# NethermindEth/cairo_zstd

Hardware: AMD Instinct MI355X
Metric: decompressed MB/s (whole node), 128 KiB-block batch (higher is better)
Workload: dtype u8

## Files before the change

cairo_zstd_amd/csrc/czstd_chain.hip:

```cpp
#include "czstd_dict.h"

#ifndef CZC_SLOTS
#define CZC_SLOTS 10
#endif
#define CZC_LPS 4
static_assert(CZC_SLOTS * CZC_LPS <= 64, "quads of one wave");
#define CZC_MAXSYM 64
#define CZC_RING 512u
#define CZC_STEPS 32u
static_assert(((CZC_STEPS * 58u + 7u) / 8u + 12u) + 12u <= 256u + 12u, "a top-up adds at most 256 bytes: one must be enough for the next group");
#define CZC_NEED ((CZC_STEPS * 58u + 7u) / 8u + 12u)
#define CZC_MAP_WORDS CZ_CHAIN_MAP_WORDS

#define CZC_E16(nb, base, xb) ((uint16_t)(((((1u << (9u - (nb))) | ((base) >> (nb))) << 6) | (xb))))
#define CZC_E16_IDLE 0x8000u

struct CzChainSlot {
    uint16_t t_ll[512], t_ml[512], t_of[256];
    union {
        struct {
            __attribute__((aligned(16))) uint8_t stage[256];
            int16_t probs[3][CZC_MAXSYM];
            uint16_t counters_ml[CZC_MAXSYM];
        };
// ... 118 lines not shown
    else if (since >= 16u) asm volatile("s_waitcnt vmcnt(16)" ::: "memory");
    else asm volatile("s_waitcnt vmcnt(0)" ::: "memory");
    asm volatile("v_accvgpr_read_b32 %0, a0\nv_accvgpr_read_b32 %1, a1\nv_accvgpr_read_b32 %2, a2\nv_accvgpr_read_b32 %3, a3\n"
                 "v_accvgpr_read_b32 %4, a4\nv_accvgpr_read_b32 %5, a5\nv_accvgpr_read_b32 %6, a6\nv_accvgpr_read_b32 %7, a7\n"
                 "v_accvgpr_read_b32 %8, a8\nv_accvgpr_read_b32 %9, a9\nv_accvgpr_read_b32 %10, a10\nv_accvgpr_read_b32 %11, a11\n"
                 "v_accvgpr_read_b32 %12, a12\nv_accvgpr_read_b32 %13, a13\nv_accvgpr_read_b32 %14, a14\nv_accvgpr_read_b32 %15, a15"
                 : "=v"(v[0].x), "=v"(v[0].y), "=v"(v[0].z), "=v"(v[0].w), "=v"(v[1].x), "=v"(v[1].y), "=v"(v[1].z), "=v"(v[1].w),
                   "=v"(v[2].x), "=v"(v[2].y), "=v"(v[2].z), "=v"(v[2].w), "=v"(v[3].x), "=v"(v[3].y), "=v"(v[3].z), "=v"(v[3].w)
                 :: "memory");
}
#else
struct CzcPre { uint4 v[CZC_PF]; };
__device__ static inline void czc_prefetch(CzcPre& pre, int has_slot, intptr_t lo, uintptr_t Sk, uintptr_t Ek) {
    const uint32_t j = (uint32_t)LANE & 3u;
    for (uint32_t r = 0; r < CZC_PF; r++) {
        const uint32_t c = j + r * CZC_LPS;
        if (has_slot) pre.v[r] = czc_load16((uintptr_t)lo - 16u * (c + 1), Sk, Ek);
    }
}
__device__ static inline void czc_pre_settle() { }
__device__ static inline void czc_pre_take(const CzcPre& pre, uint32_t, uint4* v) { for (uint32_t r = 0; r < CZC_PF; r++) v[r] = pre.v[r]; }
#endif
__device__ static inline void czc_commit(CzChainSlot& sk, int has_slot, int32_t old_lo, int32_t new_lo, const CzcPre& pre, uint32_t since) {
    const uint32_t j = (uint32_t)LANE & 3u;
    const uint32_t cnt = has_slot ? (uint32_t)(old_lo - new_lo) >> 4 : 0u;
    uint4 v[CZC_PF];
    czc_pre_take(pre, since, v);
#pragma unroll
    for (uint32_t r = 0; r < CZC_PF; r++) {
        const uint32_t c = j + r * CZC_LPS;
        if (c < cnt) {
            const uint32_t slot = ((uint32_t)old_lo - 16u * (c + 1)) & (CZC_RING - 1);
            *(uint4*)&sk.ring[slot] = v[r];
            if (slot == CZC_RING - 16) { *(uint32_t*)&sk.mirror[4] = v[r].y; *(uint32_t*)&sk.mirror[8] = v[r].z; *(uint32_t*)&sk.mirror[12] = v[r].w; }
        }
    }
}
__device__ static inline uint64_t czc_window(const CzChainSlot& sl, int32_t u) {
    const uint32_t ba = ((uint32_t)u >> 3) & (CZC_RING - 4), ph = (uint32_t)u & 31;
    const uint32_t w2 = *(const uint32_t*)(sl.ring + ba), w1 = *(const uint32_t*)(sl.ring + ba - 4), w0 = *(const uint32_t*)(sl.ring + ba - 8);
    const uint64_t hi = (((uint64_t)w2 << 32) | w1), lo = (((uint64_t)w1 << 32) | w0);
    const uint32_t h = ph ? (uint32_t)(hi >> ph) : w1, l = ph ? (uint32_t)(lo >> ph) : w0;
    return ((uint64_t)h << 32) | l;
}

struct CzcLane {
    uint32_t E;
    uint32_t S;
    int32_t  u;
    uint32_t ph;
    uint32_t w0, w1, w2;
    uint32_t slow;
};
struct CzcRole {
    const uint16_t* tb;
    const uint8_t* ringm8;
    uint32_t m1, m2;
    uint32_t sh;
    uint32_t lane0;
    uint32_t sbits;
};
#define CZC_QP(a, b, c, d) ((a) | ((b) << 2) | ((c) << 4) | ((d) << 6))
template <int CTRL> __device__ static inline uint32_t czc_qp(uint32_t v) { return (uint32_t)__builtin_amdgcn_update_dpp(0, (int)v, CTRL, 0xF, 0xF, true); }

__device__ static inline void czc_ring_words(CzcLane& c, const CzcRole& ro) {
    const uint8_t* ba = ro.ringm8 + (__builtin_amdgcn_ubfe((uint32_t)c.u, 5, 7) << 2);
    c.w0 = *(const uint32_t*)ba; c.w1 = *(const uint32_t*)(ba + 4); c.w2 = *(const uint32_t*)(ba + 8);
    c.ph = (uint32_t)c.u & 31u;
}
__device__ static inline uint32_t czc_bits32(const CzcRole& ro, uint32_t v) {
    const uint8_t* ba = ro.ringm8 + (__builtin_amdgcn_ubfe(v, 5, 7) << 2);
    return __builtin_amdgcn_alignbit(*(const uint32_t*)(ba + 8), *(const uint32_t*)(ba + 4), v & 31u);
}
#define CZC_WIDE_STEPS 16u
static_assert((CZC_WIDE_STEPS * 89u + 7u) / 8u + 12u <= CZC_NEED && CZC_STEPS % CZC_WIDE_STEPS == 0, "a redone asm group is whole wide groups, each within the staged bytes");
__device__ static inline void czc_step(CzcLane& c, const CzcRole& ro, CZ_GLOBAL uint64_t* rec, int act, int last, int store) {
    const uint32_t n = (uint32_t)__builtin_clz(c.E);
    const uint32_t x = __builtin_amdgcn_ubfe(c.E, 16, 5);
    const uint32_t p = (n << 8) + x;
    const uint32_t T = p + czc_qp<CZC_QP(1, 2, 0, 3)>(p) + czc_qp<CZC_QP(2, 0, 1, 3)>(p);
    const uint32_t t1 = czc_qp<CZC_QP(0, 0, 0, 0)>(p) & ro.m1, t2 = czc_qp<CZC_QP(1, 1, 1, 1)>(p) & ro.m2;
    const uint32_t incl = (t1 + t2 + p) >> 8;
    const uint32_t a_ = T & 0xFFu;
    const uint32_t xh = czc_bits32(ro, (uint32_t)c.u - a_);
    const uint32_t bits = __builtin_amdgcn_ubfe(xh, (0u - incl) & 31u, n);
    const uint32_t window = czc_bits32(ro, (uint32_t)c.u);
    const uint32_t cS = c.S << ro.sh;
    const uint32_t H = cS + czc_qp<CZC_QP(1, 2, 0, 3)>(cS) + czc_qp<CZC_QP(2, 0, 1, 3)>(cS);
    if (act) {
        if (store) *rec = a_ <= 32 ? ((uint64_t)window | ((uint64_t)H << 32))
                                   : ((uint64_t)((uint32_t)c.u - ro.sbits) | ((uint64_t)(H | CZC_REC_WIDE) << 32));
        if (last) c.u -= (int32_t)a_;
        else {
            c.S = (((c.E >> 22) << n) | bits) & 511u;
            c.E = (uint32_t)ro.tb[c.S] << 16;
            c.u -= (int32_t)(a_ + (T >> 8));
        }
        czc_ring_words(c, ro);
    }
}

#if defined(__HIP_DEVICE_COMPILE__)
#define CZC_ASM_STORE(OFF) "global_store_dwordx4 %[RP], v[120:123], off offset:" #OFF "\n"
#define CZC_ASM_RING01 "ds_read2_b32 v[124:125], v115 offset1:1\n"
#define CZC_ASM_LGKM_E "s_waitcnt lgkmcnt(2)\n"

#define CZC_ASM2_HEAD(WIN) \
    CZC_ASM_LGKM_E \
    "v_ffbh_u32 v100, %[E]\n" \
    "v_bfe_u32 v101, %[E], 16, 5\n" \
    "v_lshl_or_b32 v102, v100, 8, v101\n" \
    "v_lshrrev_b32 v131, 22, %[E]\n" \
    "v_and_b32_dpp v106, v100, %[M1] quad_perm:[0,0,0,0] row_mask:0xf bank_mask:0xf\n" \
    "v_and_b32_dpp v107, v100, %[M2] quad_perm:[1,1,1,1] row_mask:0xf bank_mask:0xf\n" \
    "v_add_u32_dpp v105, v102, v102 quad_perm:[1,2,0,3] row_mask:0xf bank_mask:0xf\n" \
    "v_add_u32_dpp v105, v102, v105 quad_perm:[2,0,1,3] row_mask:0xf bank_mask:0xf\n" \
    "v_add3_u32 v109, v106, v107, v105\n" \
    "s_waitcnt lgkmcnt(0)\n" \
    "v_alignbit_b32 " WIN ", %[W2], v125, %[U]\n" \
    "v_alignbit_b32 v128, v125, v124, %[U]\n" \
    "v_mov_b32 v129, " WIN "\n" \
    "v_lshlrev_b64 v[128:129], v109, v[128:129]\n" \
    "v_mov_b32 v130, v129\n" \
    "v_lshlrev_b64 v[132:133], v100, v[130:131]\n" \
    "v_lshl_add_u32 v117, v133, 1, %[TB]\n" \
    "ds_read_u16_d16_hi %[E], v117\n"
#define CZC_ASM2_TAIL(STORE, NEXTH) \
    STORE \
    "v_lshl_add_u32 v118, v133, %[SH], %[NK]\n" \
    "v_dot4c_i32_i8_e32 %[U], 0xffff, v105\n" \
    "v_max_u32_sdwa %[SLOW], %[SLOW], v105 dst_sel:DWORD dst_unused:UNUSED_PAD src0_sel:DWORD src1_sel:BYTE_0\n"    \
    "v_add_u32_dpp " NEXTH ", v118, v118 quad_perm:[1,2,0,3] row_mask:0xf bank_mask:0xf\n" \
    "v_add_u32_dpp " NEXTH ", v118, " NEXTH " quad_perm:[2,0,1,3] row_mask:0xf bank_mask:0xf\n" \
    "v_bfe_u32 v114, %[U], 5, 7\n" \
    "v_lshl_add_u32 v115, v114, 2, %[RB]\n" \
    CZC_ASM_RING01 \
    "ds_read_b32 %[W2], v115 offset:8\n"
#define CZC_ASM2_EVEN(OFF) CZC_ASM2_HEAD("v120") CZC_ASM2_TAIL("", "v123")
#define CZC_ASM2_ODD(OFF) CZC_ASM2_HEAD("v122") CZC_ASM2_TAIL(CZC_ASM_STORE(OFF), "v121")
#define CZC_ASM2_PAIR(A) CZC_ASM2_EVEN(A) CZC_ASM2_ODD(A)
__device__ static inline void czc_group_asm2(CzcLane& c, const CzcRole& ro, CZ_GLOBAL uint64_t* rec) {
    static_assert(CZC_STEPS == 32, "the asm block is unrolled for 32 steps");
    const uint32_t tb32 = (uint32_t)(uintptr_t)(__attribute__((address_space(3))) const uint16_t*)ro.tb;
    const uint32_t rb32 = (uint32_t)(uintptr_t)(__attribute__((address_space(3))) const uint8_t*)ro.ringm8;
    const uint32_t tbm = tb32 - 1024u, nk = 0u - (512u << ro.sh);
    c.S += 512u;
    asm volatile(
        "v_mov_b32 v124, %[W0]\n"
        "v_mov_b32 v125, %[W1]\n"
        "v_mov_b32 v133, %[S]\n"
        "v_lshl_add_u32 v118, %[S], %[SH], %[NK]\n"
        "s_nop 1\n"
        "v_add_u32_dpp v121, v118, v118 quad_perm:[1,2,0,3] row_mask:0xf bank_mask:0xf\n"
        "v_add_u32_dpp v121, v118, v121 quad_perm:[2,0,1,3] row_mask:0xf bank_mask:0xf\n"
        CZC_ASM2_PAIR(0) CZC_ASM2_PAIR(16) CZC_ASM2_PAIR(32) CZC_ASM2_PAIR(48) CZC_ASM2_PAIR(64) CZC_ASM2_PAIR(80) CZC_ASM2_PAIR(96) CZC_ASM2_PAIR(112)
        CZC_ASM2_PAIR(128) CZC_ASM2_PAIR(144) CZC_ASM2_PAIR(160) CZC_ASM2_PAIR(176) CZC_ASM2_PAIR(192) CZC_ASM2_PAIR(208) CZC_ASM2_PAIR(224) CZC_ASM2_PAIR(240)
        "s_waitcnt lgkmcnt(0)\n"
        "v_and_b32 %[PH], 31, %[U]\n"
        "v_mov_b32 %[W0], v124\n"
        "v_mov_b32 %[W1], v125\n"
        "v_mov_b32 %[S], v133\n"
        : [E] "+v"(c.E), [S] "+v"(c.S), [U] "+v"(c.u), [PH] "+v"(c.ph), [W0] "+v"(c.w0), [W1] "+v"(c.w1), [W2] "+v"(c.w2), [SLOW] "+v"(c.slow)
        : [TB] "v"(tbm), [RB] "v"(rb32), [M1] "v"(ro.m1 ? 0xFFu : 0u), [M2] "v"(ro.m2 ? 0xFFu : 0u), [SH] "v"(ro.sh), [NK] "v"(nk), [RP] "v"(rec)
        : "memory",
          "v100", "v101", "v102", "v105", "v106", "v107", "v109", "v114", "v115", "v117", "v118", "v120", "v121", "v122", "v123", "v124", "v125",
          "v128", "v129", "v130", "v131", "v132", "v133");
    c.S -= 512u;
}

#define CZC_ASMW_HEAD(WIN) \
    "s_waitcnt lgkmcnt(2)\n" \
    "v_ffbh_u32 v100, %[E]\n" \
    "v_and_or_b32 v101, %[E], %[XM], %[K64]\n" \
    "v_sub_u32 v102, v101, v100\n" \
    "v_lshrrev_b32 v103, 22, %[E]\n" \
    "v_sub_u32 v119, %[U], %[SB]\n"                \
    "v_add_u32_dpp v105, v102, v102 quad_perm:[1,2,0,3] row_mask:0xf bank_mask:0xf\n" \
    "v_and_b32_dpp v106, v102, %[M1] quad_perm:[0,0,0,0] row_mask:0xf bank_mask:0xf\n" \
    "v_and_b32_dpp v107, v102, %[M2] quad_perm:[1,1,1,1] row_mask:0xf bank_mask:0xf\n" \
    "v_add_u32_dpp v105, v102, v105 quad_perm:[2,0,1,3] row_mask:0xf bank_mask:0xf\n" \
    "v_add3_u32 v109, v106, v107, v102\n" \
    "v_bfe_u32 v108, v105, 16, 8\n" \
    "s_waitcnt lgkmcnt(0)\n" \
    "v_cmp_ge_u32 vcc, %[PH], v108\n" \
    "v_sub_u32 v110, %[PH], v108\n" \
    "v_alignbit_b32 " WIN ", v127, v126, %[PH]\n" \
    "v_cndmask_b32 v111, v126, v127, vcc\n" \
    "v_cndmask_b32 v112, v125, v126, vcc\n" \
    "v_cmp_gt_i32 vcc, %[N32], v110\n"             \
    "v_cmp_lt_u32_e64 s[12:13], 32, v108\n" \
    "s_nop 0\n" \
    "v_cndmask_b32 v111, v111, v125, vcc\n" \
    "v_cndmask_b32 v112, v112, v124, vcc\n" \
    "v_alignbit_b32 v113, v111, v112, v110\n" \
    "v_bfe_u32 v116, v113, v109, v100\n" \
    "v_lshl_or_b32 %[S], v103, v100, v116\n" \
    "v_lshl_add_u32 v117, %[S], 1, %[TB]\n" \
    "ds_read_u16_d16_hi %[E], v117\n"
#define CZC_ASMW_TAIL(STORE, WIN, H, NEXTH) \
    "v_cndmask_b32_e64 " WIN ", " WIN ", v119, s[12:13]\n" \
    "v_cndmask_b32_e64 v128, 0, %[FL], s[12:13]\n" \
    "v_or_b32 " H ", " H ", v128\n" \
    STORE \
    "v_lshl_add_u32 v118, %[S], %[SH], %[NK]\n" \
    "v_dot4c_i32_i8_e32 %[U], 0x01ff0001, v105\n" \
    "v_and_b32 v129, 31, v108\n" \
    "v_add_u32_dpp " NEXTH ", v118, v118 quad_perm:[1,2,0,3] row_mask:0xf bank_mask:0xf\n" \
    "v_add_u32_dpp " NEXTH ", v118, " NEXTH " quad_perm:[2,0,1,3] row_mask:0xf bank_mask:0xf\n" \
    "v_bfe_u32 v114, %[U], 5, 7\n" \
    "v_and_b32 %[PH], 31, %[U]\n" \
    "v_lshl_add_u32 v115, v114, 2, %[RB]\n" \
    "ds_read2_b32 v[124:125], v115 offset1:1\n" \
    "ds_read2_b32 v[126:127], v115 offset0:2 offset1:3\n"
#define CZC_ASMW_EVEN(OFF) CZC_ASMW_HEAD("v120") CZC_ASMW_TAIL("", "v120", "v121", "v123")
#define CZC_ASMW_ODD(OFF) CZC_ASMW_HEAD("v122") CZC_ASMW_TAIL(CZC_ASM_STORE(OFF), "v122", "v123", "v121")
#define CZC_ASMW_PAIR(A) CZC_ASMW_EVEN(A) CZC_ASMW_ODD(A)
__device__ static inline void czc_group_asm_wide(CzcLane& c, const CzcRole& ro, CZ_GLOBAL uint64_t* rec) {
    const uint32_t tb32 = (uint32_t)(uintptr_t)(__attribute__((address_space(3))) const uint16_t*)ro.tb;
    const uint32_t rb32 = (uint32_t)(uintptr_t)(__attribute__((address_space(3))) const uint8_t*)ro.ringm8 - 4u;
    const uint32_t tbm = tb32 - 1024u, nk = 0u - (512u << ro.sh), k64 = ro.lane0 ? 0x40000040u : 0x40u;
    c.S += 512u;
    asm volatile(
        "v_bfe_u32 v114, %[U], 5, 7\n"
        "v_lshl_add_u32 v115, v114, 2, %[RB]\n"
        "ds_read2_b32 v[124:125], v115 offset1:1\n"
        "ds_read2_b32 v[126:127], v115 offset0:2 offset1:3\n"
        "v_lshl_add_u32 v118, %[S], %[SH], %[NK]\n"
        "s_nop 1\n"
        "v_add_u32_dpp v121, v118, v118 quad_perm:[1,2,0,3] row_mask:0xf bank_mask:0xf\n"
        "v_add_u32_dpp v121, v118, v121 quad_perm:[2,0,1,3] row_mask:0xf bank_mask:0xf\n"
        CZC_ASMW_PAIR(0) CZC_ASMW_PAIR(16) CZC_ASMW_PAIR(32) CZC_ASMW_PAIR(48) CZC_ASMW_PAIR(64) CZC_ASMW_PAIR(80) CZC_ASMW_PAIR(96) CZC_ASMW_PAIR(112)
        CZC_ASMW_PAIR(128) CZC_ASMW_PAIR(144) CZC_ASMW_PAIR(160) CZC_ASMW_PAIR(176) CZC_ASMW_PAIR(192) CZC_ASMW_PAIR(208) CZC_ASMW_PAIR(224) CZC_ASMW_PAIR(240)
        "s_waitcnt lgkmcnt(0)\n"
        : [E] "+v"(c.E), [S] "+v"(c.S), [U] "+v"(c.u), [PH] "+v"(c.ph)
        : [TB] "v"(tbm), [RB] "v"(rb32), [M1] "v"(ro.m1 ? 0xFFu : 0u), [M2] "v"(ro.m2 ? 0xFFu : 0u), [SH] "v"(ro.sh), [NK] "v"(nk), [K64] "v"(k64),
          [SB] "v"(ro.sbits), [FL] "v"(CZC_REC_WIDE), [XM] "s"(0x1F0000u), [N32] "s"(-32), [RP] "v"(rec)
        : "memory", "vcc", "s12", "s13",
          "v100", "v101", "v102", "v103", "v105", "v106", "v107", "v108", "v109", "v110", "v111", "v112", "v113", "v114", "v115",
          "v116", "v117", "v118", "v119", "v120", "v121", "v122", "v123", "v124", "v125", "v126", "v127", "v128", "v129");
    c.S -= 512u;
    czc_ring_words(c, ro);
}
#endif

#ifdef CZ_PROFILE
#define CZC_PROF_ACC(i) do { const unsigned long long n_ = __builtin_amdgcn_s_memtime(); cprof[i] += n_ - ct_; ct_ = n_; } while (0)
#define CZC_PROF_CNT(i) do { cprof[i] += 1; } while (0)
#else
#define CZC_PROF_ACC(i) do { } while (0)
#define CZC_PROF_CNT(i) do { } while (0)
#endif
#define CZC_LO_DEAD (-(1 << 30))
#define CZC_NSEQ_DEAD 0xFFFFFFFFu
#if defined(__HIP_DEVICE_COMPILE__)
__device__ static inline bool czc_any(bool b) { return __builtin_amdgcn_ballot_w64(b) != 0; }
#else
__device__ static inline bool czc_any(bool b) { return __ballot(b ? 1 : 0) != 0; }
#endif
__device__ static inline uint32_t czc_q0(uint32_t v) { return (uint32_t)__shfl((int)v, LANE & ~3); }
__device__ static inline uint64_t czc_q0_64(uint64_t v) { return ((uint64_t)czc_q0((uint32_t)(v >> 32)) << 32) | czc_q0((uint32_t)v); }

struct CzsBlk { uint32_t type, blk_off, bsize;
                uint32_t lt, regen, lit_hdr, nseq, sbody, modes; };
struct CzsWalk { const uint8_t* src; uint64_t len, pos, end, h8; uint32_t h8sh, defined, has_checksum; int first, active, ok, have_tree; };
__device__ static inline uint64_t czs_ld8_issue(const uint8_t* src, uint64_t len, uint64_t at, uint32_t* sh) {
    const uint64_t a2 = at + 8 <= len ? at : len - 8;
    uint64_t v; __builtin_memcpy(&v, src + a2, 8);
    *sh = (uint32_t)(at - a2);
    return v;
}
__device__ static inline uint64_t czs_ld8_value(uint64_t raw, uint32_t sh) { return sh >= 8 ? 0 : raw >> (8 * sh); }
__device__ static inline uint64_t czs_ld8(const uint8_t* src, uint64_t len, uint64_t at) { uint32_t sh; const uint64_t v = czs_ld8_issue(src, len, at, &sh); return czs_ld8_value(v, sh); }
__device__ static inline void czs_begin(CzsWalk& w, const uint8_t* src, uint64_t len, int valid) {
    w.src = src; w.len = len; w.pos = 0; w.end = 0; w.h8 = 0; w.h8sh = 8; w.defined = 0; w.has_checksum = 0; w.first = 1; w.active = 0; w.ok = 0; w.have_tree = 0;
    if (!valid || len < 8 || len >= 0xFFFFFFF0ull) return;
    const uint64_t h0 = czs_ld8(src, len, 0);
    const uint32_t magic = (uint32_t)h0;
    const uint32_t d = (uint32_t)(h0 >> 32) & 0xFF;
    const uint32_t single = (d >> 5) & 1, didf = d & 3, dl = didf == 3 ? 4 : didf, flag = d >> 6;
    const uint32_t fl = flag == 0 ? (single ? 1u : 0u) : flag == 1 ? 2u : flag == 2 ? 4u : 8u;
    const uint32_t hl = 5 + (single ? 0 : 1) + dl + fl;
    if (magic != 0xFD2FB528u || len < hl) return;
    if (!single) { const uint32_t wd = (uint32_t)(h0 >> 40) & 0xFF; const uint64_t base = 1ull << (10 + (wd >> 3)); if (base + (base / 8) * (wd & 7) >= 4123168604160ull) return; }
    w.pos = hl; w.active = 1; w.has_checksum = (d >> 2) & 1; w.h8 = czs_ld8_issue(src, len, hl, &w.h8sh);
}
__device__ static inline void czs_dict_check(CzsWalk& w, const cz_dict_entry* dicts, uint32_t ndicts) {
    if (!w.active) return;
    const uint64_t h0 = czs_ld8(w.src, w.len, 0);
    const uint32_t d = (uint32_t)(h0 >> 32) & 0xFF, didf = d & 3, dl = didf == 3 ? 4 : didf, at = 5 + (((d >> 5) & 1) ? 0 : 1);
    uint32_t id = (uint32_t)(h0 >> (8 * at));
    if (at + dl > 8) id |= (uint32_t)(czs_ld8(w.src, w.len, 8) << (8 * (8 - at)));
    id = dl == 0 ? 0u : (dl == 4 ? id : id & ((1u << (8 * dl)) - 1u));
    if (cz_dict_find(dicts, ndicts, id) == CZ_DICT_UNKNOWN) { w.active = 0; w.ok = 0; }
}
__device__ static inline int czs_next(CzsWalk& w, uint32_t chain_min_nseq, CzsBlk& b) {
    const uint8_t* src = w.src; const uint64_t len = w.len;
    if (!w.active) return 0;
    do {
        uint64_t pos = w.pos;
        if (pos == ~0ull) { w.active = 0; w.ok = 1; return 0; }
        if (len - pos < 3) break;
        const uint64_t h = czs_ld8_value(w.h8, w.h8sh);
        const uint32_t b0 = (uint32_t)h & 0xFF, b1 = (uint32_t)(h >> 8) & 0xFF, b2 = (uint32_t)(h >> 16) & 0xFF;
        const uint32_t type = (b0 >> 1) & 3, size = (b0 >> 3) | (b1 << 5) | (b2 << 13), blast = b0 & 1;
        if (type == 3 || size > 128u * 1024u) break;
        const uint64_t body = pos + 3; const uint32_t content = type == 1 ? 1u : size;
        if (len - body < content) break;
        w.pos = blast ? ~0ull : body + content;
        if (blast) w.end = body + content;
        else w.h8 = czs_ld8_issue(src, len, body + content, &w.h8sh);
        b.type = type; b.blk_off = (uint32_t)body; b.bsize = size; b.lt = 0; b.regen = 0; b.lit_hdr = 0; b.nseq = 0; b.sbody = 0; b.modes = 0;
        if (type != 2) return 1;
        if (size == 0) break;
        const uint32_t l0 = (uint32_t)(h >> 24) & 0xFF, lt = l0 & 3, fmt = (l0 >> 2) & 3;
        const uint32_t need = lt <= 1 ? ((fmt == 0 || fmt == 2) ? 1u : (fmt == 1 ? 2u : 3u)) : (fmt <= 1 ? 3u : (fmt == 2 ? 4u : 5u));
        if (size < need) break;
        const uint32_t l1 = need > 1 ? (uint32_t)(h >> 32) & 0xFF : 0, l2 = need > 2 ? (uint32_t)(h >> 40) & 0xFF : 0, l3 = need > 3 ? (uint32_t)(h >> 48) & 0xFF : 0, l4 = need > 4 ? (uint32_t)(h >> 56) & 0xFF : 0;
        uint32_t upper, regen;
        if (lt <= 1) { regen = (fmt == 0 || fmt == 2) ? l0 >> 3 : (fmt == 1 ? (l0 >> 4) + (l1 << 4) : (l0 >> 4) + (l1 << 4) + (l2 << 12)); upper = lt == 1 ? 1u : regen; }
        else {
            regen = fmt <= 1 ? (l0 >> 4) + ((l1 & 0x3f) << 4) : (fmt == 2 ? (l0 >> 4) + (l1 << 4) + ((l2 & 3) << 12) : (l0 >> 4) + (l1 << 4) + ((l2 & 0x3f) << 12));
            upper = fmt <= 1 ? (l1 >> 6) + (l2 << 2) : (fmt == 2 ? (l2 >> 2) + (l3 << 6) : (l2 >> 6) + (l3 << 2) + (l4 << 10));
        }
        if (size - need < upper) break;
        if (lt == 3 && !w.have_tree) break;
        if (lt == 2) w.have_tree = 1;
        const uint32_t so = need + upper, sl_ = size - so;
        if (sl_ == 0) break;
        const uint64_t sq = czs_ld8(src, len, body + so);
        const uint32_t s0 = (uint32_t)sq & 0xFF, s1 = (uint32_t)(sq >> 8) & 0xFF, s2 = (uint32_t)(sq >> 16) & 0xFF;
        uint32_t n = 0, hb = 0;
        if (s0 == 0) { }
        else if (s0 <= 127) { if (sl_ < 2) break; n = s0; hb = 1; }
        else if (s0 <= 254) { if (sl_ < 3) break; n = ((s0 - 128) << 8) + s1; hb = 2; }
        else { if (sl_ < 4) break; n = s1 + (s2 << 8) + 0x7F00u; hb = 3; }
        b.lt = lt; b.regen = regen; b.lit_hdr = need;
        if (!n) return 1;
        if (w.first && n < chain_min_nseq) break;
        b.nseq = n; b.modes = (uint32_t)(sq >> (8 * hb)) & 0xFF; b.sbody = so + hb + 1;
        int undefined = 0;
        for (int t = 0; t < 3; t++) {
// ... 205 lines not shown
        const unsigned long long wm = __ballot(wx);
        if (wm) {
            uint32_t base = 0;
            if (LANE == __ffsll((long long)wm) - 1) base = atomicAdd(&a.scan_ctl[206], (uint32_t)__popcll(wm));
            base = (uint32_t)__shfl((int)base, __ffsll((long long)wm) - 1);
            if (wx) a.wx_list[base + (uint32_t)__popcll(wm & ((1ull << LANE) - 1ull))] = f;
        }
    }
    if (with_lits) {
        const unsigned long long todo = __ballot(valid && !(a.frame_pre[f < a.n ? f : 0] & CZ_PRE_DONE));
        if (LANE == 0 && todo) atomicAdd(&a.scan_ctl[204], (uint32_t)__popcll(todo));
    }
}

__device__ static inline __attribute__((always_inline)) int czc_parse_tables(cz_gcptr blk, uint32_t bsize, uint32_t sbody, uint32_t modes, uint32_t want, const uint8_t* stage, uint32_t stage_n,
                                       int16_t (*probs)[CZC_MAXSYM], uint32_t* info, int32_t* rle, uint32_t* bitoff) {
    uint32_t off = sbody;
    for (int t = 0; t < 3; t++) {
        const uint32_t md = (modes >> (6 - 2 * t)) & 3, max_log = t == 1 ? 8u : 9u;
        const int take = (want >> t) & 1u;
        if (md == 0) {
            if (take) {
                const int8_t* d = t == 0 ? CZ_LL_DEFAULT : t == 1 ? CZ_OF_DEFAULT : CZ_ML_DEFAULT;
                const uint32_t n = t == 0 ? 36u : t == 1 ? 29u : 53u, lg = t == 1 ? 5u : 6u;
                for (uint32_t s = 0; s < n; s++) probs[t][s] = d[s];
                *info = (*info & ~(0x3FFu << (10 * t))) | (((n - 1) | (lg << 6)) << (10 * t));
                rle[t] = -1;
            }
        } else if (md == 1) {
            if (off >= bsize) return 1;
            const uint32_t sym = blk[off]; off += 1;
            if (take) {
                if (sym >= (t == 0 ? 36u : (t == 1 ? 32u : 53u))) return 1;
                rle[t] = (int32_t)sym; *info &= ~(0x3FFu << (10 * t));
            }
        } else if (md == 2) {
            CzFBits br; br.g = (cz_gcptr)(blk + off); br.len = bsize - off; br.idx = 0; br.stage = stage; br.stage_lo = 0; br.stage_hi = 0;
            if (stage && off - sbody < stage_n) { br.stage = stage + (off - sbody); br.stage_hi = stage_n - (off - sbody); }
            uint32_t np, lg, used;
            const int into = take ? t : (want & 2u ? 1 : 2);
            if (cz_fse_read_probs_inl(br, max_log, probs[into], &np, &lg, &used, 100, CZC_MAXSYM) || np > CZC_MAXSYM || np == 0) return 1;
            if (take) { *info = (*info & ~(0x3FFu << (10 * t))) | (((np - 1) | (lg << 6)) << (10 * t)); rle[t] = -1; }
            off += used;
            if (off > bsize) return 1;
        }
        if ((want >> (t + 1)) == 0) break;
    }
    *bitoff = off;
    return 0;
}

#define CZC_SYNC() cz_wave_sync()
extern "C" __global__ void __launch_bounds__(CZ_WG_THREADS, 1) cz_chain_kernel(cz_batch_args a) {
    __shared__ CzChainShared cs;
    __builtin_amdgcn_s_setprio(3);
    for (uint32_t i = (uint32_t)LANE; i < 36; i += 64) cs.llml[i] = CZ_LL_BASE[i] | ((uint32_t)CZ_LL_BITS[i] << 24);
    for (uint32_t i = (uint32_t)LANE; i < 53; i += 64) cs.llml[40 + i] = CZ_ML_BASE[i] | ((uint32_t)CZ_ML_BITS[i] << 24);
    if (LANE < 2) cs.idle[LANE] = (uint16_t)CZC_E16_IDLE;
    __syncthreads();
    const uint32_t qk = (uint32_t)LANE >> 2, ql = (uint32_t)LANE & 3u;
    const int has_slot = qk < CZC_SLOTS;
    const int owner = has_slot && ql == 0;
    CzChainSlot& sl = cs.slot[has_slot ? qk : 0];
    CzcRole ro;
    ro.ringm8 = sl.ring - 8; ro.tb = cs.idle; ro.sbits = 0;
    ro.m1 = (ql == 1 || ql == 2) ? 0xFF00u : 0u; ro.m2 = ql == 2 ? 0xFF00u : 0u; ro.sh = ql == 3 ? 0u : 9u * ql; ro.lane0 = ql == 0;
    const uint16_t* my_table = ql == 0 ? sl.t_ll : (ql == 1 ? sl.t_ml : sl.t_of);
#ifdef CZ_PROFILE
    unsigned long long cprof[16] = {0, 0, 0, 0, 0, 0, 0, 0, 0, 0, 0, 0, 0, 0, 0, 0}, ct_ = __builtin_amdgcn_s_memtime();
#endif
    uint32_t ndesc = 0, nlarge = 0; for (int c = 0; c < 20; c++) { ndesc += a.scan_ctl[c]; if ((uint32_t)c >= CZ_BIG_BLOCK_CLASS) nlarge += a.scan_ctl[c]; }
    if (ndesc > a.blk_capacity) ndesc = a.blk_capacity;
    if (nlarge > ndesc) nlarge = ndesc;
    const uint32_t list_lo = a.chain_part == 2u ? nlarge : 0u, list_hi = a.chain_part == 1u ? nlarge : ndesc;
    uint32_t* const list_counter = a.chain_part == 2u ? &a.scan_ctl[212] : &a.scan_ctl[64];
    const int publish = a.chain_part == 1u;
    if (list_lo >= list_hi) { if (LANE == 0) atomicAdd(&a.scan_ctl[205], 1u); return; }
    int chain_live = 0, wide = 0, exhausted = owner ? 0 : 1;
    uint32_t qnseq = CZC_NSEQ_DEAD, done = 0, sbits = 0;
    uintptr_t S = 0, E = 0; intptr_t ring_base = 0;
    int32_t lo_rel = CZC_LO_DEAD;
    CZ_GLOBAL uint64_t* rec = nullptr;
    CZ_GLOBAL uint64_t* const sink = (CZ_GLOBAL uint64_t*)(a.chain_arena + 8);
    CZ_GLOBAL uint64_t* rp = sink; uint32_t rp_step = 0;
    (void)rp;
    uint32_t o_frame = 0, o_nseq = 0, o_mapflags = 0, o_bitoff = 0, o_bad0 = 0; uint64_t o_hdr = 0; int o_have = 0, o_pub = 0;
    CzcLane c; c.E = (uint32_t)CZC_E16_IDLE << 16; c.S = 0; c.u = 0; c.ph = 0; c.w0 = c.w1 = c.w2 = 0; c.slow = 0;
    CzcPre pre = {};
    uint32_t since = 0;
    for (;;) {
        if (czc_any((o_have | exhausted) == 0)) {
            cz_gcptr blk = nullptr; uint32_t bsize = 0, sbody = 0, modes = 0; uint32_t def[3] = {0, 0, 0};
            int got = 0;
            if (owner && !o_have && !exhausted) {
                for (;;) {
                    const uint32_t idx = list_lo + atomicAdd(list_counter, 1u);
                    if (idx >= list_hi) { exhausted = 1; break; }
                    const cz_blk_desc d = a.blk_desc[idx];
                    if (!d.nseq) continue;
                    blk = (cz_gcptr)(a.in_base + a.in_off[d.frame] + d.blk_off); bsize = d.bsize; sbody = d.sbody; modes = d.modes;
                    def[0] = d.def[0]; def[1] = d.def[1]; def[2] = d.def[2];
                    o_frame = d.frame; o_nseq = d.nseq; o_hdr = d.hdr; o_have = 1; got = 1;
                    o_pub = publish && (a.frame_pre[d.frame] & CZ_PRE_WXBIG) != 0u;
                    break;
                }
            }
            {
                const uintptr_t base = (uintptr_t)blk + sbody;
                const uintptr_t bk = (uintptr_t)czc_q0_64((uint64_t)base), Sk = (uintptr_t)czc_q0_64((uint64_t)(uintptr_t)blk), Ek = Sk + czc_q0(bsize);
                CZC_SYNC();
                if (czc_q0((uint32_t)got) && has_slot) for (uint32_t cc = ql; cc < 16; cc += CZC_LPS) *(uint4*)&sl.stage[16 * cc] = czc_load16(bk + 16 * cc, Sk, Ek);
                CZC_SYNC();
            }
            CZC_PROF_ACC(8); CZC_PROF_CNT(13);
            uint32_t binfo = 0; int32_t rles[3] = {-1, -1, -1}; int bad = 0;
            if (got) {
                o_mapflags = 0;
                for (int t = 0; t < 3; t++) if (((modes >> (6 - 2 * t)) & 3) != 3) o_mapflags |= 1u << t;
                bad = czc_parse_tables(blk, bsize, sbody, modes, 7u, sl.stage, 256u, sl.probs, &binfo, rles, &o_bitoff);
            }
            CZC_PROF_ACC(9);
            for (int t = 0; t < 3; t++) {
                const int rep = got && !bad && ((modes >> (6 - 2 * t)) & 3) == 3;
                if (!__ballot(rep)) continue;
                cz_gcptr dblk = nullptr; uint32_t dbsize = 0, dsbody = 0, dmodes = 0;
                if (rep) {
                    if (def[t] >= ndesc) bad = 1;
                    else {
                        const cz_blk_desc dd = a.blk_desc[def[t]];
                        if (dd.frame != o_frame) bad = 1;
                        else { dblk = (cz_gcptr)(a.in_base + a.in_off[dd.frame] + dd.blk_off); dbsize = dd.bsize; dsbody = dd.sbody; dmodes = dd.modes; }
                    }
                }
                const int go = rep && !bad;
                {
                    const uintptr_t base = (uintptr_t)dblk + dsbody;
                    const uintptr_t bk = (uintptr_t)czc_q0_64((uint64_t)base), Sk = (uintptr_t)czc_q0_64((uint64_t)(uintptr_t)dblk), Ek = Sk + czc_q0(dbsize);
                    CZC_SYNC();
                    if (czc_q0((uint32_t)go) && has_slot) for (uint32_t cc = ql; cc < 16; cc += CZC_LPS) *(uint4*)&sl.stage[16 * cc] = czc_load16(bk + 16 * cc, Sk, Ek);
                    CZC_SYNC();
                }
                if (go) { uint32_t dummy; bad = czc_parse_tables(dblk, dbsize, dsbody, dmodes, 1u << t, sl.stage, 256u, sl.probs, &binfo, rles, &dummy); }
            }
            if (got && bad) { got = 0; o_have = 0; a.frame_first[o_frame] = 0; if (o_pub) CZ_ST_AGENT(&a.chain_arena[o_hdr + 3], (uint64_t)2); }
            if (got && a.exec_counter) {
                const uint32_t info = (binfo >> 10) & 0x3FFu, lg = info >> 6, np = (info & 63u) + 1u, n6 = (o_nseq + 63u) >> 6;
                uint32_t nearc = 0, farc = 0;
                if (rles[1] >= 0) { nearc = rles[1] >= 2 && rles[1] <= 13 ? 256u : 0u; farc = rles[1] >= 14 ? 256u : 0u; }
                else if (lg) {
                    for (uint32_t sy = 2; sy < np; sy++) { const int32_t pr = sl.probs[1][sy]; const uint32_t cnt = pr > 0 ? (uint32_t)pr : (pr < 0 ? 1u : 0u); if (sy <= 13u) nearc += cnt; else farc += cnt; }
                    nearc = (nearc << 8) >> lg; farc = (farc << 8) >> lg;
                }
                if (nearc) atomicAdd(a.chain_top + 5, (unsigned long long)nearc * n6);
                if (farc) atomicAdd(a.chain_top + 6, (unsigned long long)farc * n6);
                uint32_t longc = 0;
                for (int t = 0; t < 3; t += 2) {
                    const uint32_t inf = (binfo >> (10 * t)) & 0x3FFu, lgt = inf >> 6, npt = (inf & 63u) + 1u, lim = t == 0 ? 8u : 13u;
                    if (rles[t] >= 0) longc += (uint32_t)rles[t] > lim ? 256u : 0u;
                    else if (lgt) {
                        uint32_t cl = 0;
                        for (uint32_t sy = lim + 1u; sy < npt; sy++) { const int32_t pr = sl.probs[t][sy]; cl += pr > 0 ? (uint32_t)pr : 0u; }
                        longc += (cl << 8) >> lgt;
                    }
                }
                if (longc) atomicAdd(a.chain_top + 7, (unsigned long long)longc * n6);
            }
            CZC_PROF_ACC(10);
            {
                CZC_SYNC();
                int tbad = 0;
                for (unsigned long long need = __ballot(owner && got); need; need &= need - 1) {
                    const int ol = cz_unii(__ffsll((long long)need) - 1);
                    const uint32_t binf = cz_readlane(binfo, ol), mf = cz_readlane(o_mapflags, ol);
                    const uint64_t hk = ((uint64_t)cz_readlane((uint32_t)(o_hdr >> 32), ol) << 32) | cz_readlane((uint32_t)o_hdr, ol);
                    CzChainSlot& bs = cs.slot[(uint32_t)ol >> 2];
                    cz_gptr maps = (cz_gptr)(a.chain_arena + hk + 4);
                    int sbad = 0;
#pragma unroll 1
                    for (uint32_t o = 0; o < 3; o++) {
                        const uint32_t bk = o == 0 ? 0u : (o == 1 ? 2u : 1u);
                        const uint32_t info = (binf >> (10 * bk)) & 0x3FFu;
                        if (!(info >> 6)) continue;
                        uint16_t* table = bk == 0 ? bs.t_ll : (bk == 1 ? bs.t_of : bs.t_ml);
                        uint8_t* symof = bk == 1 ? bs.stage : (uint8_t*)bs.t_of;
                        cz_gptr map = !((mf >> bk) & 1u) ? (cz_gptr)nullptr : (bk == 0 ? maps : (bk == 2 ? maps + 512 : maps + 1024));
                        sbad |= czc_fse_build_wave(table, bs.probs[bk], (info & 63u) + 1u, info >> 6, symof, bs.counters_ml, cs.llml, bk, map);
                        cz_wave_sync();
                    }
                    if (sbad && LANE == ol) tbad = 1;
                }
                CZC_SYNC();
                if (got && tbad) { got = 0; o_have = 0; a.frame_first[o_frame] = 0; if (o_pub) CZ_ST_AGENT(&a.chain_arena[o_hdr + 3], (uint64_t)2); }
                if (got) for (int t = 0; t < 3; t++) if (rles[t] >= 0) {
                    uint16_t* table = t == 0 ? sl.t_ll : (t == 1 ? sl.t_of : sl.t_ml);
                    table[0] = CZC_E16(0u, 0u, t == 1 ? (uint32_t)rles[t] : (cs.llml[(t == 2 ? 40u : 0u) + (uint32_t)rles[t]] >> 24));
                    if ((o_mapflags >> t) & 1u) ((cz_gptr)(a.chain_arena + o_hdr + 4))[t == 0 ? 0 : (t == 2 ? 512 : 1024)] = (uint8_t)rles[t];
                }
                CZC_SYNC();
            }
            CZC_PROF_ACC(11);
            const int qgot = (int)czc_q0((uint32_t)got) && has_slot;
            const uint32_t gn = czc_q0(o_nseq);
            const uintptr_t gblk = (uintptr_t)czc_q0_64((uint64_t)(uintptr_t)blk);
            const uint32_t gbitoff = czc_q0(o_bitoff), gbsize = czc_q0(bsize);
            if (qgot) {
                S = gblk + gbitoff; E = gblk + gbsize; qnseq = gn; done = 0; wide = 0;
                sbits = (uint32_t)(S & (CZC_RING - 1)) * 8u;
                ring_base = (intptr_t)(S & ~(uintptr_t)(CZC_RING - 1));
                lo_rel = (int32_t)((intptr_t)((E + 15) & ~(uintptr_t)15) - ring_base) - 256;
            }
            czc_pre_settle();
            czc_prefetch(pre, qgot, ring_base + lo_rel + 256, S, E);
            czc_commit(sl, qgot, lo_rel + 256, lo_rel, pre, 0u);
            CZC_SYNC();
            czc_prefetch(pre, qgot, ring_base + lo_rel, S, E);
            since = 0;
            int32_t u0 = 0; uint32_t st_ll = 0, st_of = 0, st_ml = 0;
            if (got) {
                int32_t p = (int32_t)(E - S) * 8; int skipped = 0;
                o_bad0 = 0;
                for (;;) {
                    const uint32_t b = p > 0 ? (uint32_t)(czc_window(sl, (int32_t)sbits + p) >> 63) : 0; p -= 1; skipped++;
                    if (b == 1 || skipped > 8) break;
                }
                if (skipped > 8) o_bad0 = 1;
                uint32_t stv[3] = {0, 0, 0};
                for (int t = 0; t < 3; t++) {
                    if (rles[t] >= 0) continue;
                    const uint32_t lg = (binfo >> (10 * t + 6)) & 15u;
                    stv[t] = p > 0 ? (uint32_t)(czc_window(sl, (int32_t)sbits + p) >> (64 - lg)) : 0; p -= (int32_t)lg;
                }
                st_ll = stv[0]; st_of = stv[1]; st_ml = stv[2];
                if (p < 0) o_bad0 = 1;
                u0 = (int32_t)sbits + p;
            }
            {
                const uint32_t qll = czc_q0(st_ll), qml = czc_q0(st_ml), qof = czc_q0(st_of), qu = czc_q0((uint32_t)u0);
                const uint64_t qh = czc_q0_64(o_hdr);
                if (qgot) {
                    c.u = (int32_t)qu; c.slow = 0; ro.sbits = sbits;
                    c.S = ql == 0 ? qll : (ql == 1 ? qml : (ql == 2 ? qof : 0u));
                    if (ql == 3) { ro.tb = cs.idle; c.S = 0; } else ro.tb = my_table;
                    c.E = (uint32_t)ro.tb[c.S] << 16;
                    czc_ring_words(c, ro);
                    rec = (CZ_GLOBAL uint64_t*)(a.chain_arena + qh + 4 + CZC_MAP_WORDS);
                    if (ql < 3) { rp = rec; rp_step = CZC_STEPS; }
                    chain_live = 1;
                }
            }
            CZC_PROF_ACC(1);
        }
        if (!czc_any(chain_live != 0)) { if (!czc_any(exhausted == 0)) break; continue; }
        {
            const int32_t uq = (int32_t)czc_qp<CZC_QP(0, 0, 0, 0)>((uint32_t)c.u);
            const int32_t cur = ((uq > 0 ? uq : 1) - 1) >> 3;
            if (czc_any(cur - (int32_t)CZC_NEED < lo_rel)) {
                int32_t new_lo = chain_live ? ((cur - (int32_t)(CZC_RING - 4) + 15) & ~15) : lo_rel;
                if (new_lo > lo_rel) new_lo = lo_rel;
                if (new_lo < lo_rel - 256) new_lo = lo_rel - 256;
                CZC_SYNC();
                czc_commit(sl, chain_live, lo_rel, new_lo, pre, since);
                lo_rel = new_lo;
                CZC_SYNC();
                czc_prefetch(pre, chain_live, ring_base + lo_rel, S, E);
                since = 0;
                if (chain_live) czc_ring_words(c, ro);
                CZC_PROF_ACC(2); CZC_PROF_CNT(5);
            }
        }
        {
            const uint32_t left = qnseq - done;
            const bool tail = czc_any(left <= CZC_STEPS);
            int ran_asm = 0;
            (void)tail; (void)wide;
#if defined(__HIP_DEVICE_COMPILE__)
            if (!tail && !(a.debug_flags & CZ_DEBUG_CHAIN_CPP_STEP)) {
                bool any_wide = czc_any(wide != 0);
                if (!any_wide) {
                    const uint32_t sv_E = c.E, sv_S = c.S; const int32_t sv_u = c.u;
                    c.slow = 0;
                    czc_group_asm2(c, ro, rp);
                    since += CZC_GROUP_STORES;
                    if (czc_any(c.slow > 32)) {
                        const int hit = chain_live && ql < 3 && c.slow > 32;
                        wide |= (int)czc_q0((uint32_t)hit);
                        c.E = sv_E; c.S = sv_S; c.u = sv_u; czc_ring_words(c, ro);
                        any_wide = true;
                    }
                }
                if (any_wide) { czc_group_asm_wide(c, ro, rp); since += CZC_GROUP_STORES; }
                if (chain_live) done += CZC_STEPS;
                rp += rp_step;
                ran_asm = 1;
            }
#endif
            if (!ran_asm) {
                const uint32_t steps = !chain_live ? 0u : (left < CZC_WIDE_STEPS ? left : CZC_WIDE_STEPS);
                for (uint32_t i = 0; i < CZC_WIDE_STEPS; i++) czc_step(c, ro, rec + done + i, i < steps, done + i + 1 == qnseq, ql == 0);
                done += steps;
                if (rp_step) rp += steps;
            }
            CZC_PROF_ACC(3); CZC_PROF_CNT(6);
        }
        if (czc_any(done >= qnseq)) {
            const int fin = chain_live && done >= qnseq;
            int fbad = 0;
            if (fin && owner) {
                fbad = o_bad0 || c.u - (int32_t)sbits != 0;
                if (fbad) a.frame_first[o_frame] = 0;
                else { uint64_t* h = a.chain_arena + o_hdr; h[0] = ((uint64_t)o_nseq << 32) | o_mapflags; h[1] = o_bitoff; if (!o_pub) h[3] = 0; }
                o_have = 0;
            }
            if (__ballot(fin && owner && o_pub)) {
                CZ_RELEASE_AGENT();
                if (fin && owner && o_pub) CZ_ST_AGENT(&a.chain_arena[o_hdr + 3], (uint64_t)(fbad ? 2 : 1));
            }
            if (fin) { chain_live = 0; wide = 0; ro.tb = cs.idle; c.S = 0; c.E = (uint32_t)CZC_E16_IDLE << 16; rp = sink; rp_step = 0; qnseq = CZC_NSEQ_DEAD; done = 0; lo_rel = CZC_LO_DEAD; }
            CZC_PROF_ACC(4);
        }
    }
#ifdef CZ_PROFILE
    if (LANE == 0 && a.prof) { for (int i = 0; i < 8; i++) atomicAdd(&a.prof[32 + i], cprof[i]); for (int i = 8; i < 14; i++) atomicAdd(&a.prof[50 + i - 8], cprof[i]); }
#endif
    if (LANE == 0) atomicAdd(&a.scan_ctl[205], 1u);
}
```

Baseline: 180,400.

## Run several asm sequence groups back-to-back inside one asm block

```diff
diff --git a/cairo_zstd_amd/csrc/czstd_chain.hip b/cairo_zstd_amd/csrc/czstd_chain.hip
--- a/cairo_zstd_amd/csrc/czstd_chain.hip
+++ b/cairo_zstd_amd/csrc/czstd_chain.hip
@@ -224,6 +224,7 @@
     const uint32_t t1 = czc_qp<CZC_QP(0, 0, 0, 0)>(p) & ro.m1, t2 = czc_qp<CZC_QP(1, 1, 1, 1)>(p) & ro.m2;
     const uint32_t incl = (t1 + t2 + p) >> 8;
     const uint32_t a_ = T & 0xFFu;
+    if (act && a_ > c.slow) c.slow = a_;
     const uint32_t xh = czc_bits32(ro, (uint32_t)c.u - a_);
     const uint32_t bits = __builtin_amdgcn_ubfe(xh, (0u - incl) & 31u, n);
     const uint32_t window = czc_bits32(ro, (uint32_t)c.u);
@@ -281,11 +282,13 @@
 #define CZC_ASM2_EVEN(OFF) CZC_ASM2_HEAD("v120") CZC_ASM2_TAIL("", "v123")
 #define CZC_ASM2_ODD(OFF) CZC_ASM2_HEAD("v122") CZC_ASM2_TAIL(CZC_ASM_STORE(OFF), "v121")
 #define CZC_ASM2_PAIR(A) CZC_ASM2_EVEN(A) CZC_ASM2_ODD(A)
-__device__ static inline void czc_group_asm2(CzcLane& c, const CzcRole& ro, CZ_GLOBAL uint64_t* rec) {
+struct CzcSaved { uint32_t E, S; int32_t u; };
+__device__ static inline uint32_t czc_run_asm2(CzcLane& c, const CzcRole& ro, CZ_GLOBAL uint64_t*& rp, uint64_t rp_bytes, int32_t lim, uint32_t k, CzcSaved& sv) {
     static_assert(CZC_STEPS == 32, "the asm block is unrolled for 32 steps");
     const uint32_t tb32 = (uint32_t)(uintptr_t)(__attribute__((address_space(3))) const uint16_t*)ro.tb;
     const uint32_t rb32 = (uint32_t)(uintptr_t)(__attribute__((address_space(3))) const uint8_t*)ro.ringm8;
     const uint32_t tbm = tb32 - 1024u, nk = 0u - (512u << ro.sh);
+    uint32_t kleft = k;
     c.S += 512u;
     asm volatile(
         "v_mov_b32 v124, %[W0]\n"
@@ -295,19 +298,38 @@
         "s_nop 1\n"
         "v_add_u32_dpp v121, v118, v118 quad_perm:[1,2,0,3] row_mask:0xf bank_mask:0xf\n"
         "v_add_u32_dpp v121, v118, v121 quad_perm:[2,0,1,3] row_mask:0xf bank_mask:0xf\n"
+        "v_mov_b32 %[SLOW], 0\n"
+        "Lczc_run_top_%=:\n"
+        "v_mov_b32_dpp v100, %[U] quad_perm:[0,0,0,0] row_mask:0xf bank_mask:0xf\n"
+        "v_cmp_gt_i32 vcc, %[LIM], v100\n"
+        "s_cbranch_vccnz Lczc_run_out_%=\n"
+        "v_mov_b32 %[SVE], %[E]\n"
+        "v_mov_b32 %[SVS], v133\n"
+        "v_mov_b32 %[SVU], %[U]\n"
+        "v_mov_b32 %[SLOW], 0\n"
         CZC_ASM2_PAIR(0) CZC_ASM2_PAIR(16) CZC_ASM2_PAIR(32) CZC_ASM2_PAIR(48) CZC_ASM2_PAIR(64) CZC_ASM2_PAIR(80) CZC_ASM2_PAIR(96) CZC_ASM2_PAIR(112)
         CZC_ASM2_PAIR(128) CZC_ASM2_PAIR(144) CZC_ASM2_PAIR(160) CZC_ASM2_PAIR(176) CZC_ASM2_PAIR(192) CZC_ASM2_PAIR(208) CZC_ASM2_PAIR(224) CZC_ASM2_PAIR(240)
+        "v_cmp_lt_u32 vcc, 32, %[SLOW]\n"
+        "s_cbranch_vccnz Lczc_run_out_%=\n"
+        "v_lshl_add_u64 %[RP], %[RP], 0, %[RPB]\n"
+        "s_sub_u32 %[K], %[K], 1\n"
+        "s_cmp_lg_u32 %[K], 0\n"
+        "s_cbranch_scc1 Lczc_run_top_%=\n"
+        "Lczc_run_out_%=:\n"
         "s_waitcnt lgkmcnt(0)\n"
         "v_and_b32 %[PH], 31, %[U]\n"
         "v_mov_b32 %[W0], v124\n"
         "v_mov_b32 %[W1], v125\n"
         "v_mov_b32 %[S], v133\n"
-        : [E] "+v"(c.E), [S] "+v"(c.S), [U] "+v"(c.u), [PH] "+v"(c.ph), [W0] "+v"(c.w0), [W1] "+v"(c.w1), [W2] "+v"(c.w2), [SLOW] "+v"(c.slow)
-        : [TB] "v"(tbm), [RB] "v"(rb32), [M1] "v"(ro.m1 ? 0xFFu : 0u), [M2] "v"(ro.m2 ? 0xFFu : 0u), [SH] "v"(ro.sh), [NK] "v"(nk), [RP] "v"(rec)
-        : "memory",
+        : [E] "+v"(c.E), [S] "+v"(c.S), [U] "+v"(c.u), [PH] "+v"(c.ph), [W0] "+v"(c.w0), [W1] "+v"(c.w1), [W2] "+v"(c.w2), [SLOW] "=&v"(c.slow),
+          [RP] "+v"(rp), [K] "+s"(kleft), [SVE] "=&v"(sv.E), [SVS] "=&v"(sv.S), [SVU] "=&v"(sv.u)
+        : [TB] "v"(tbm), [RB] "v"(rb32), [M1] "v"(ro.m1 ? 0xFFu : 0u), [M2] "v"(ro.m2 ? 0xFFu : 0u), [SH] "v"(ro.sh), [NK] "v"(nk), [RPB] "v"(rp_bytes), [LIM] "v"(lim)
+        : "memory", "vcc", "scc",
           "v100", "v101", "v102", "v105", "v106", "v107", "v109", "v114", "v115", "v117", "v118", "v120", "v121", "v122", "v123", "v124", "v125",
           "v128", "v129", "v130", "v131", "v132", "v133");
     c.S -= 512u;
+    sv.S -= 512u;
+    return k - kleft;
 }
 
 #define CZC_ASMW_HEAD(WIN) \
@@ -399,6 +421,36 @@
 #else
 __device__ static inline bool czc_any(bool b) { return __ballot(b ? 1 : 0) != 0; }
 #endif
+#define CZC_RUN_CAP ((CZC_RING - CZC_NEED) / CZC_STEPS)
+static_assert(CZC_RUN_CAP >= 2 && CZC_RUN_CAP <= 16, "a short, bounded run");
+__device__ static inline int32_t czc_topup_lim(int32_t lo_rel) {
+    const int32_t L = lo_rel + (int32_t)CZC_NEED;
+    return L > 0 ? 8 * L + 1 : INT32_MIN;
+}
+__device__ static inline uint32_t czc_run_len(uint32_t left) {
+    if (!czc_any(left <= CZC_STEPS * CZC_RUN_CAP)) return CZC_RUN_CAP;
+    uint32_t k = 0;
+    while (k < CZC_RUN_CAP && !czc_any(left <= CZC_STEPS * (k + 1u))) k++;
+    return k;
+}
+#if !defined(__HIP_DEVICE_COMPILE__)
+struct CzcSaved { uint32_t E, S; int32_t u; };
+__device__ static inline uint32_t czc_run_cpp(CzcLane& c, const CzcRole& ro, CZ_GLOBAL uint64_t*& rp, uint64_t rp_bytes, int32_t lim, uint32_t k, CzcSaved& sv,
+                                              int live, int store) {
+    uint32_t kleft = k;
+    c.slow = 0;
+    do {
+        if (czc_any((int32_t)czc_qp<CZC_QP(0, 0, 0, 0)>((uint32_t)c.u) < lim)) break;
+        sv.E = c.E; sv.S = c.S; sv.u = c.u; c.slow = 0;
+        for (uint32_t i = 0; i < CZC_STEPS; i++) czc_step(c, ro, rp + i, live, 0, store);
+        if (czc_any(c.slow > 32)) break;
+        rp = (CZ_GLOBAL uint64_t*)((uintptr_t)rp + (uintptr_t)rp_bytes);
+        kleft -= 1;
+    } while (kleft != 0);
+    return k - kleft;
+}
+#endif
+
 __device__ static inline uint32_t czc_q0(uint32_t v) { return (uint32_t)__shfl((int)v, LANE & ~3); }
 __device__ static inline uint64_t czc_q0_64(uint64_t v) { return ((uint64_t)czc_q0((uint32_t)(v >> 32)) << 32) | czc_q0((uint32_t)v); }
 
@@ -770,8 +822,8 @@
     int32_t lo_rel = CZC_LO_DEAD;
     CZ_GLOBAL uint64_t* rec = nullptr;
     CZ_GLOBAL uint64_t* const sink = (CZ_GLOBAL uint64_t*)(a.chain_arena + 8);
-    CZ_GLOBAL uint64_t* rp = sink; uint32_t rp_step = 0;
-    (void)rp;
+    CZ_GLOBAL uint64_t* rp = sink; uint64_t rp_bytes = 0;
+    int32_t run_lim = czc_topup_lim(lo_rel);
     uint32_t o_frame = 0, o_nseq = 0, o_mapflags = 0, o_bitoff = 0, o_bad0 = 0; uint64_t o_hdr = 0; int o_have = 0, o_pub = 0;
     CzcLane c; c.E = (uint32_t)CZC_E16_IDLE << 16; c.S = 0; c.u = 0; c.ph = 0; c.w0 = c.w1 = c.w2 = 0; c.slow = 0;
     CzcPre pre = {};
@@ -895,7 +947,7 @@
                 S = gblk + gbitoff; E = gblk + gbsize; qnseq = gn; done = 0; wide = 0;
                 sbits = (uint32_t)(S & (CZC_RING - 1)) * 8u;
                 ring_base = (intptr_t)(S & ~(uintptr_t)(CZC_RING - 1));
-                lo_rel = (int32_t)((intptr_t)((E + 15) & ~(uintptr_t)15) - ring_base) - 256;
+                lo_rel = (int32_t)((intptr_t)((E + 15) & ~(uintptr_t)15) - ring_base) - 256; run_lim = czc_topup_lim(lo_rel);
             }
             czc_pre_settle();
             czc_prefetch(pre, qgot, ring_base + lo_rel + 256, S, E);
@@ -932,7 +984,7 @@
                     c.E = (uint32_t)ro.tb[c.S] << 16;
                     czc_ring_words(c, ro);
                     rec = (CZ_GLOBAL uint64_t*)(a.chain_arena + qh + 4 + CZC_MAP_WORDS);
-                    if (ql < 3) { rp = rec; rp_step = CZC_STEPS; }
+                    if (ql < 3) { rp = rec; rp_bytes = CZC_STEPS * 8u; }
                     chain_live = 1;
                 }
             }
@@ -948,7 +1000,7 @@
                 if (new_lo < lo_rel - 256) new_lo = lo_rel - 256;
                 CZC_SYNC();
                 czc_commit(sl, chain_live, lo_rel, new_lo, pre, since);
-                lo_rel = new_lo;
+                lo_rel = new_lo; run_lim = czc_topup_lim(lo_rel);
                 CZC_SYNC();
                 czc_prefetch(pre, chain_live, ring_base + lo_rel, S, E);
                 since = 0;
@@ -957,36 +1009,51 @@
             }
         }
         {
-            const uint32_t left = qnseq - done;
-            const bool tail = czc_any(left <= CZC_STEPS);
-            int ran_asm = 0;
-            (void)tail; (void)wide;
+            const bool tail = czc_any(qnseq - done <= CZC_STEPS);
+            int ran = 0;
 #if defined(__HIP_DEVICE_COMPILE__)
-            if (!tail && !(a.debug_flags & CZ_DEBUG_CHAIN_CPP_STEP)) {
+            const bool runs = !(a.debug_flags & CZ_DEBUG_CHAIN_CPP_STEP);
+#else
+            const bool runs = true;
+#endif
+            if (!tail && runs) {
                 bool any_wide = czc_any(wide != 0);
                 if (!any_wide) {
-                    const uint32_t sv_E = c.E, sv_S = c.S; const int32_t sv_u = c.u;
-                    c.slow = 0;
-                    czc_group_asm2(c, ro, rp);
-                    since += CZC_GROUP_STORES;
+                    const uint32_t k = czc_run_len(qnseq - done);
+                    CzcSaved sv;
+#if defined(__HIP_DEVICE_COMPILE__)
+                    const uint32_t g = czc_run_asm2(c, ro, rp, rp_bytes, run_lim, k, sv);
+#else
+                    const uint32_t g = czc_run_cpp(c, ro, rp, rp_bytes, run_lim, k, sv, chain_live, ql == 0);
+#endif
+                    if (chain_live) done += CZC_STEPS * g;
+                    since += CZC_GROUP_STORES * g;
+                    ran = 1;
                     if (czc_any(c.slow > 32)) {
                         const int hit = chain_live && ql < 3 && c.slow > 32;
                         wide |= (int)czc_q0((uint32_t)hit);
-                        c.E = sv_E; c.S = sv_S; c.u = sv_u; czc_ring_words(c, ro);
+                        c.E = sv.E; c.S = sv.S; c.u = sv.u; czc_ring_words(c, ro);
+                        since += CZC_GROUP_STORES;
                         any_wide = true;
                     }
                 }
-                if (any_wide) { czc_group_asm_wide(c, ro, rp); since += CZC_GROUP_STORES; }
-                if (chain_live) done += CZC_STEPS;
-                rp += rp_step;
-                ran_asm = 1;
-            }
+#if defined(__HIP_DEVICE_COMPILE__)
+                if (any_wide) {
+                    czc_group_asm_wide(c, ro, rp); since += CZC_GROUP_STORES;
+                    if (chain_live) done += CZC_STEPS;
+                    rp = (CZ_GLOBAL uint64_t*)((uintptr_t)rp + (uintptr_t)rp_bytes);
+                    ran = 1;
+                }
+#else
+                if (any_wide) ran = 0;
 #endif
-            if (!ran_asm) {
+            }
+            if (!ran) {
+                const uint32_t left = qnseq - done;
                 const uint32_t steps = !chain_live ? 0u : (left < CZC_WIDE_STEPS ? left : CZC_WIDE_STEPS);
                 for (uint32_t i = 0; i < CZC_WIDE_STEPS; i++) czc_step(c, ro, rec + done + i, i < steps, done + i + 1 == qnseq, ql == 0);
                 done += steps;
-                if (rp_step) rp += steps;
+                if (rp_bytes) rp += steps;
             }
             CZC_PROF_ACC(3); CZC_PROF_CNT(6);
         }
@@ -1003,7 +1070,7 @@
                 CZ_RELEASE_AGENT();
                 if (fin && owner && o_pub) CZ_ST_AGENT(&a.chain_arena[o_hdr + 3], (uint64_t)(fbad ? 2 : 1));
             }
-            if (fin) { chain_live = 0; wide = 0; ro.tb = cs.idle; c.S = 0; c.E = (uint32_t)CZC_E16_IDLE << 16; rp = sink; rp_step = 0; qnseq = CZC_NSEQ_DEAD; done = 0; lo_rel = CZC_LO_DEAD; }
+            if (fin) { chain_live = 0; wide = 0; ro.tb = cs.idle; c.S = 0; c.E = (uint32_t)CZC_E16_IDLE << 16; rp = sink; rp_bytes = 0; qnseq = CZC_NSEQ_DEAD; done = 0; lo_rel = CZC_LO_DEAD; run_lim = czc_topup_lim(lo_rel); }
             CZC_PROF_ACC(4);
         }
     }
```

Measured after the change: 182,000, median of 6. No clear change (+0.9%).
